# thekingofkings/embedding

Measured on AMD Instinct MI355X. Metric: SGNS training edges/sec, higher is better.
Workload: dtype f32

## Files before the change

embedding_amd/_native.py:

```python
import ctypes as C
import os

_HERE = os.path.dirname(os.path.abspath(__file__))
LIB_PATH = os.path.join(_HERE, "libdge.so")

DGE_OK, DGE_ERR_ARG, DGE_ERR_RANGE, DGE_ERR_TOPK, DGE_ERR_CAP, DGE_ERR_STATE, DGE_ERR_DEVICE, DGE_ERR_IO = range(8)


class DgeError(RuntimeError):
    def __init__(self, code, msg):
        super().__init__("libdge error %d: %s" % (code, msg))
        self.code = code


class TrainConfig(C.Structure):
    _fields_ = [
        ("dim", C.c_int32), ("window", C.c_int32), ("negative", C.c_int32), ("min_count", C.c_int32),
        ("epochs", C.c_int32), ("workers", C.c_int32), ("alpha", C.c_float), ("min_alpha", C.c_float),
        ("seed", C.c_uint64), ("table_size", C.c_int64), ("n_vertices", C.c_int32), ("update_policy", C.c_int32),
        ("use_hs", C.c_int32), ("reserved", C.c_int32),
    ]


class TrainStats(C.Structure):
# ... 242 lines not shown
    "dge_names_count": (_int, [_vp, _P(_i64)]),
    "dge_names_cstrs": (_int, [_vp, _P(_vp)]),
    "dge_names_free": (None, [_vp]),
    "dge_walks_from_seq_text": (_int, [_int, _vp, _i64, _vp, _int, _P(_vp), _P(SeqInfo)]),
    "dge_walks_from_seq_files": (_int, [_int, _vp, _i32, _vp, _int, _P(_vp), _P(SeqInfo)]),
    "dge_walks_to_seq_text": (_int, [_vp, _i64, _i64, _vp, _int, _vp, _i64, _P(_i64), _P(SeqOutInfo)]),
    "dge_walks_write_seq": (_int, [_vp, _i64, _i64, _vp, _int, C.c_char_p, _int, _P(SeqOutInfo)]),
    "dge_walks_to_host": (_int, [_vp, _vp, _i64]),
    "dge_walks_info": (_int, [_vp, _P(_i64), _P(_i32), _P(_vp)]),
    "dge_walks_add_position_prefix": (_int, [_vp, _i32]),
    "dge_walks_free": (None, [_vp]),
    "dge_count_tokens": (_int, [_vp, _i64, _i64, _i32, _vp]),
    "dge_model_create": (_int, [_int, _P(TrainConfig), _vp, _P(_vp)]),
    "dge_model_set_stream": (_int, [_vp, _vp]),
    "dge_model_train": (_int, [_vp, _vp, _i64, _i64, _i64, _i32, _i64, _dbl, _i64]),
    "dge_train_sgns": (_int, [_int, _vp, _i64, _i32, _P(TrainConfig), _P(_vp)]),
    "dge_train_sgns_device": (_int, [_vp, _P(TrainConfig), _P(_vp)]),
    "dge_model_walk_and_train": (_int, [_vp, _vp, _vp, _i64, _i64, _i64, _i64, _i32, _i64, _dbl, _i64]),
    "dge_model_vectors": (_int, [_vp, _P(_vp), _P(_vp), _P(_i64), _P(_i32)]),
    "dge_model_syn1neg": (_int, [_vp, _P(_vp)]),
    "dge_model_syn1": (_int, [_vp, _P(_vp), _P(_i64)]),
    "dge_model_huffman": (_int, [_vp, _P(_vp), _P(_vp), _P(_vp)]),
    "dge_model_counts": (_int, [_vp, _P(_vp)]),
    "dge_model_table": (_int, [_vp, _P(_vp), _P(_i64)]),
    "dge_model_stats": (_int, [_vp, _P(TrainStats)]),
    "dge_model_row_rates": (_int, [_vp, _P(C.c_double), _P(C.c_double), _P(C.c_double), _P(C.c_double)]),
    "dge_model_table_placement": (_int, [_vp, _i32, _vp, _vp, _vp]),
    "dge_model_table_runs": (_int, [_vp, _vp, _vp]),
    "dge_model_tune_placement": (_int, [_vp, _vp, _i64, _i64, _i32, _vp, _vp, _vp]),
    "dge_model_placement_search": (_int, [_vp, _vp, _vp, _vp, _vp]),
    "dge_model_reset_stats": (_int, [_vp]),
    "dge_model_schedule": (_int, [_vp, _P(_i32), _P(_i64), _P(_i32)]),
    "dge_model_kernel": (_int, [_vp, C.c_char_p, _i32]),
    "dge_model_lock_stats": (_int, [_vp, _P(_i64), _P(_i64), _P(_i64)]),
    "dge_model_score_pairs": (_int, [_vp, _vp, _vp, _i64, _vp]),
    "dge_model_eval_links": (_int, [_vp, _vp, _i64, _i64, _i32, C.c_uint64, _P(EvalResult)]),
    "dge_model_eval_sgns": (_int, [_vp, _vp, _i64, _i64, C.c_uint64, _P(EvalResult)]),
    "dge_write_vec": (_int, [_vp, _vp, C.c_char_p, _int]),
    "dge_model_free": (None, [_vp]),
    "dge_model_set_partition": (_int, [_vp, _i32, _i32, _i32]),
    "dge_model_partition_floats": (_int, [_vp, _i32, _P(_i64)]),
    "dge_model_export_partition": (_int, [_vp, _int, _i32, _i32, _vp]),
    "dge_model_import_partition": (_int, [_vp, _int, _i32, _i32, _vp]),
    "dge_model_export_partition_async": (_int, [_vp, _int, _i32, _i32, _vp, _vp]),
    "dge_model_import_partition_async": (_int, [_vp, _int, _i32, _i32, _vp, _vp]),
    "dge_model_stream": (_int, [_vp, _P(_vp)]),
    "dge_host_sync_count": (_int, [_P(_i64)]),
    "dge_model_sync_size": (_int, [_vp, _P(_i64)]),
    "dge_model_snapshot": (_int, [_vp]),
    "dge_model_export_delta": (_int, [_vp, _vp]),
    "dge_model_import_delta": (_int, [_vp, _vp, C.c_float]),
    "dge_comm_unique_id": (_int, [_vp]),
    "dge_comm_create": (_int, [_P(_vp), _vp, _int, _int, _int]),
    "dge_comm_free": (None, [_vp]),
    "dge_model_allreduce_deltas": (_int, [_vp, _vp]),
    "dge_model_ring_pass": (_int, [_vp, _vp, _i32]),
    "dge_model_gather_table": (_int, [_vp, _vp, _int]),
    "dge_set_tuning": (_int, [_i32, _i64]),
    "dge_get_tuning": (_int, [_i32, _vp]),
    "dge_ndcg_at_k": (_int, [_int, _vp, _i32, _vp, _i32, _i32, _i32, _P(_dbl), _P(_dbl)]),
    "dge_knn_cosine": (_int, [_int, _vp, _i32, _i32, _i32, _vp, _vp, _P(_dbl)]),
    "dge_vectors_from_vec_text": (_int, [_int, _vp, _i64, _int, _vp, _int, _P(_vp), _P(VecInfo)]),
    "dge_vectors_from_vec_files": (_int, [_int, _vp, _i32, _int, _vp, _int, _P(_vp), _P(VecInfo)]),
    "dge_vectors_from_host": (_int, [_int, _vp, _i64, _i32, _vp, _P(_vp)]),
    "dge_vectors_info": (_int, [_vp, _P(_i64), _P(_i32), _P(_vp), _P(_vp)]),
    "dge_vectors_to_host": (_int, [_vp, _vp, _vp, _i64]),
# ... 72 lines not shown
```

embedding_amd/csrc/sgns.hip:

```cpp
#include <hipcub/hipcub.hpp>
#include <math.h>
#include <stdlib.h>
#include <string.h>

#include <algorithm>
#include <limits>
#include <string>

#include "dge_algos.h"
#include "dge_internal.h"
#include "sgns_kernels.h"
#include "sgns_model.h"

std::atomic<int64_t> g_dge_tuning[DGE_TUNE_COUNT];
namespace { struct TuningInit { TuningInit() { for (auto& k : g_dge_tuning) k.store(-1); } } g_tuning_init; }
std::atomic<int64_t> g_dge_host_syncs{0};
extern "C" int dge_host_sync_count(int64_t* n) {
    if (!n) DGE_FAIL(DGE_ERR_ARG, "dge_host_sync_count: null output");
    *n = g_dge_host_syncs.load(std::memory_order_relaxed);
    return DGE_OK;
}
extern "C" int dge_set_tuning(int32_t knob, int64_t value) {
    if (knob < 0 || knob >= DGE_TUNE_COUNT) DGE_FAIL(DGE_ERR_ARG, "dge_set_tuning: unknown knob %d", knob);
    g_dge_tuning[knob] = value < 0 ? -1 : value;
// ... 584 lines not shown
    if (n_exceptions) *n_exceptions = m->n_exc;
    return DGE_OK;
}

extern "C" int dge_model_schedule(const dge_model* m, int32_t* update_policy, int64_t* workers, int32_t* hot_rows) {
    if (!m) DGE_FAIL(DGE_ERR_ARG, "dge_model_schedule: null model");
    if (!m->has_plan) DGE_FAIL(DGE_ERR_STATE, "dge_model_schedule: nothing has been trained yet");
    if (update_policy) *update_policy = m->last_plan.reported_policy();
    if (workers) *workers = m->last_plan.workers;
    if (hot_rows) *hot_rows = m->last_plan.hot_rows;
    return DGE_OK;
}

extern "C" int dge_model_lock_stats(const dge_model* mc, int64_t* pairs_put_back, int64_t* rounds_short, int64_t* rounds) {
    dge_model* m = const_cast<dge_model*>(mc);
    if (!m) DGE_FAIL(DGE_ERR_ARG, "dge_model_lock_stats: null model");
    DGE_HIP(hipSetDevice(m->device));
    DGE_HIP(hipStreamSynchronize(m->stream));
    unsigned long long c[3] = {0, 0, 0};
    DGE_HIP(hipMemcpy(c, m->d_counters + 4, sizeof(c), hipMemcpyDeviceToHost));
    if (pairs_put_back) *pairs_put_back = (int64_t)c[0];
    if (rounds_short) *rounds_short = (int64_t)c[1];
    if (rounds) *rounds = (int64_t)c[2];
    return DGE_OK;
}

extern "C" int dge_model_kernel(const dge_model* m, char* buf, int32_t cap) {
    if (!m || !buf || cap <= 0) DGE_FAIL(DGE_ERR_ARG, "dge_model_kernel: bad argument");
    if (!m->has_plan) DGE_FAIL(DGE_ERR_STATE, "dge_model_kernel: nothing has been trained yet");
    snprintf(buf, (size_t)cap, "%s", m->last_plan.kernel_name().c_str());
    return DGE_OK;
}

extern "C" int dge_model_reset_stats(dge_model* m) {
    if (!m) DGE_FAIL(DGE_ERR_ARG, "dge_model_reset_stats: null model");
    int rc = dge_drain_events(m);
    if (rc) return rc;
    DGE_HIP(hipMemsetAsync(m->d_counters, 0, 2 * sizeof(unsigned long long), m->stream));
    DGE_HIP(hipMemsetAsync(m->d_counters + 4, 0, 3 * sizeof(unsigned long long), m->stream));
    DGE_HIP(hipStreamSynchronize(m->stream));
    m->kernel_ms = 0; m->walk_ms = 0; m->launches = 0;
    return DGE_OK;
}

extern "C" int dge_model_set_partition(dge_model* m, int32_t n_parts, int32_t ctx_part, int32_t tgt_part) {
    if (!m) DGE_FAIL(DGE_ERR_ARG, "dge_model_set_partition: null model");
    if (n_parts <= 1) { m->part_n = 1; m->part_ctx = 0; m->part_tgt = 0; return DGE_OK; }
    if (ctx_part < 0 || ctx_part >= n_parts || tgt_part < 0 || tgt_part >= n_parts) DGE_FAIL(DGE_ERR_ARG, "dge_model_set_partition: partition out of range");
    if (m->V < n_parts) DGE_FAIL(DGE_ERR_ARG, "dge_model_set_partition: %d partitions for %lld vocabulary rows", n_parts, (long long)m->V);
    m->part_n = n_parts; m->part_ctx = ctx_part; m->part_tgt = tgt_part;
    return DGE_OK;
}
```

embedding_amd/csrc/sgns_kernels.h:

```cpp
#pragma once
#include <hip/hip_runtime.h>
#include <stdint.h>

#include "dge_algos.h"
#include "dge_internal.h"
#include "sgns_plan.h"

#define EXP_TABLE_SIZE 1000
#define MAX_EXP 6
#define NEG_BATCH 5

struct TrainParams {
    const int32_t* sen; const int64_t* len; const int64_t* wb;
    float* syn0; float* syn1neg;
    int32_t acc_rows, acc_drain;
    const uint4* ctab;
    const double* run_base; const uint32_t* run_row; const uint32_t* exc_slot; const int32_t* exc_row;
    int32_t n_runs, n_exc;
    double T_inv;
    const float* exp_table;
    int64_t n_rows; int32_t L, W, K, stride;
    int32_t D;
    int64_t V, T;
    uint64_t T_magic, W_magic;
// ... 1150 lines not shown
            l1.v[q].x += neu.v[q].x; l1.v[q].y += neu.v[q].y; l1.v[q].z += neu.v[q].z; l1.v[q].w += neu.v[q].w;
        }
        if (HOTMIX && (last < hot_rows || p.syn0_free)) {
            if (use_mb) lk_post<DCH>(s_mb, s_mb_flag, wk, n_posts, 2, lane == 0 ? last : -1, 1.0f, neu, lane);
            else rowA_atomic_axpy<DCH>(syn0, last, lane, 1.0f, neu);
        } else {
            rowA_store<DCH, 16, BIG>(l1, syn0, last, lane);
            row_commit_wait(STRICT ? row_probe_lines(syn0, last, lane, DCH * 2) : 0.f);
            if (lane == 14) row_unlock<STRICT>(locks0, last);
        }
        my_pairs++;
        if (PART) {
            pair_mask &= pair_mask - 1ull;
            c = first_bit_from(pair_mask, 0, c_hi + 1);
        } else {
            c++;
            if (c == i) c++;
        }
    }
    LK_CLOSE_CENTRE();
    if (pend_row >= 0 && !flushA_blocking<DCH, STRICT, BIG, HOTMIX>(syn1neg, locks1, pend_row, my_dh + (cur_buf ^ 1) * DCH * 64 + lane, lane, hot_rows, WD ? &s_deadline : nullptr)) LK_GIVE_UP();
#undef LK_TOK
#undef LK_POSITIVE
#undef LK_CLOSE_CENTRE
#undef LK_GIVE_UP
    if (lane == 0) {
        if (my_pairs) atomicAdd(&p.counters[0], my_pairs);
        if (my_words) atomicAdd(&p.counters[1], my_words);
        if (PART) { atomicAdd(&p.counters[4], (unsigned long long)n_aborted); atomicAdd(&p.counters[5], (unsigned long long)n_short); atomicAdd(&p.counters[6], (unsigned long long)n_rounds); }
        if (use_mb) __hip_atomic_fetch_add(&s_mb_done, 1, __ATOMIC_RELEASE, __HIP_MEMORY_SCOPE_WORKGROUP);
    }
}

#define HSW_NQ (DCH <= 2 ? 6 : 3)
template <int DCH>
__device__ __forceinline__ void hot_addA(float* s_hot, int* s_cnt, int slot, int drain, const TableView& t, int32_t row, int lane, const Row<DCH>& x) {
    float* a = s_hot + slot * (DCH * 64) + 4 * lane;
#pragma unroll
    for (int c = 0; c < DCH; c++) {
        atomicAdd(a + c * 64 + 0, x.v[c].x); atomicAdd(a + c * 64 + 1, x.v[c].y); atomicAdd(a + c * 64 + 2, x.v[c].z); atomicAdd(a + c * 64 + 3, x.v[c].w);
    }
    int n = 0;
    if (lane == 0) n = atomicAdd(&s_cnt[slot], 1) + 1;
    n = __shfl(n, 0, 16);
    if (n % drain == 0) {
        float* e = s_hot + slot * (DCH * 64) + lane;
        float* gp = t.base + (size_t)row * (t.row_bytes / 4) + lane;
#pragma unroll
        for (int c = 0; c < DCH; c++)
#pragma unroll
            for (int m = 0; m < 4; m++) {
                if ((uint32_t)(c * 64 + 16 * m + lane) >= t.valid) continue;
                const float v = atomicExch(e + c * 64 + 16 * m, 0.f);
                if (v != 0.f) atomicAdd(gp + c * 64 + 16 * m, v);
            }
    }
}
template <int DCH>
__device__ __forceinline__ void row_add(Row<DCH>& y, const Row<DCH>& x) {
#pragma unroll
    for (int c = 0; c < DCH; c++) { y.v[c].x += x.v[c].x; y.v[c].y += x.v[c].y; y.v[c].z += x.v[c].z; y.v[c].w += x.v[c].w; }
}
__device__ __forceinline__ int hsw_n_copies(const TrainParams& p, int32_t nd) {
    int r = 1;
#pragma unroll
    for (int k = 1; k < HS_REP; k++) r += nd >= p.hs_rep_thr[k] ? 1 : 0;
// ... 479 lines not shown
                else hipLaunchKernelGGL((k_sgns_train<DCH, 2, BIG, true, false>), g, b, pl.shmem, st, p);
            } else if (pl.part) hipLaunchKernelGGL((k_sgns_train<DCH, 2, BIG, false, true>), g, b, 0, st, p);
            else hipLaunchKernelGGL((k_sgns_train<DCH, 2, BIG, false, false>), g, b, 0, st, p);
            break;
        case TrainForm::HsCentre:
            if constexpr (DCH <= 4 && !BIG) {
                if (!pl.nlock) hipLaunchKernelGGL((k_sgns_train_hsw<DCH, false, 3>), g, b, pl.shmem, st, p);
                else if (pl.waves == 3) {
                    if (pl.head) hipLaunchKernelGGL((k_sgns_train_hsw<DCH, true, 3, true>), g, b, pl.shmem, st, p);
                    else hipLaunchKernelGGL((k_sgns_train_hsw<DCH, true, 3>), g, b, pl.shmem, st, p);
                } else if constexpr (DCH <= 2) {
                    if (pl.head) {
                        (void)hipFuncSetAttribute((const void*)k_sgns_train_hsw<DCH, true, 7, true>, hipFuncAttributeMaxDynamicSharedMemorySize, (int)pl.shmem);
                        hipLaunchKernelGGL((k_sgns_train_hsw<DCH, true, 7, true>), g, b, pl.shmem, st, p);
                    } else {
                        (void)hipFuncSetAttribute((const void*)k_sgns_train_hsw<DCH, true, 7>, hipFuncAttributeMaxDynamicSharedMemorySize, (int)pl.shmem);
                        hipLaunchKernelGGL((k_sgns_train_hsw<DCH, true, 7>), g, b, pl.shmem, st, p);
                    }
                }
            }
            break;
        case TrainForm::Locked:
            if (pl.hotmix) {
                if (pl.part) hipLaunchKernelGGL((k_sgns_train_locked<DCH, false, BIG, true, true>), g, b, 0, st, p);
                else hipLaunchKernelGGL((k_sgns_train_locked<DCH, false, BIG, true, false>), g, b, 0, st, p);
            } else if (pl.part) {
                if (pl.wdog) hipLaunchKernelGGL((k_sgns_train_locked<DCH, false, BIG, false, true, true>), g, b, 0, st, p);
                else hipLaunchKernelGGL((k_sgns_train_locked<DCH, false, BIG, false, true>), g, b, 0, st, p);
            } else if (pl.strict) {
                if (pl.wdog) hipLaunchKernelGGL((k_sgns_train_locked<DCH, true, BIG, false, false, true>), g, b, 0, st, p);
                else hipLaunchKernelGGL((k_sgns_train_locked<DCH, true, BIG, false, false>), g, b, 0, st, p);
            } else {
                if (pl.wdog) hipLaunchKernelGGL((k_sgns_train_locked<DCH, false, BIG, false, false, true>), g, b, 0, st, p);
                else hipLaunchKernelGGL((k_sgns_train_locked<DCH, false, BIG, false, false>), g, b, 0, st, p);
            }
            break;
        default: break;
    }
}
template <int DCH>
static inline void launch_train(const TrainParams& p, const TrainPlan& pl, hipStream_t st) {
    if (pl.big) launch_train_b<DCH, true>(p, pl, st);
    else launch_train_b<DCH, false>(p, pl, st);
}
```

embedding_amd/csrc/sgns_plan.h:

```cpp
#pragma once
#include <math.h>
#include <stdarg.h>
#include <stdint.h>
#include <stdio.h>

#include <algorithm>
#include <string>
#include <vector>

#include "../../include/dge.h"

#define HS_REP 16
#define HS_REP_NODES 64
#define HS_REP_ROWS ((HS_REP - 1) * HS_REP_NODES)
#ifndef DGE_LOCKED_WAVES
#define DGE_LOCKED_WAVES 3
#endif
#ifndef DGE_HOTMIX_WAVES
#define DGE_HOTMIX_WAVES 3
#endif
#ifndef DGE_HS_WAVES
#define DGE_HS_WAVES 3
#endif

// ... 73 lines not shown
    if (memo.n == n && memo.workers == W) return memo.rows;
    const double power = 0.75, twp = s.neg_norm, tw = (double)std::max<int64_t>(s.total_words, 1);
    double tail = 0.0; int64_t H = s.V;
    const double bound = 0.2 / (5.0 * (double)W * (double)std::max(n, 1));
    while (H > 0) {
        const double c = (double)counts[H - 1];
        const double q = pow(c, power) / twp, pp = c / tw;
        if (tail + q * q + pp * pp >= bound) break;
        tail += q * q + pp * pp; H--;
    }
    int64_t Hs = 0;
    while (Hs < s.V && (double)W * (double)n * (double)counts[Hs] / tw > 0.5) Hs++;
    memo.n = n; memo.workers = W; memo.rows = std::max(H, Hs);
    return memo.rows;
}

static inline double lock_failures(const ScheduleStats& s) { return (double)((int64_t)s.n_cus * 3 * 16) * 5.0 * s.neg_collision; }
static inline bool row_share_caps_workers(const ScheduleStats& s) { return (int64_t)(48.0 / std::max(s.row_share_max, 1e-12)) < 4096; }
static inline bool locks_work(const ScheduleStats& s) { return s.V >= 131072 && lock_failures(s) < 0.4; }
static inline bool tables_need_segments(const ScheduleStats& s) { return (uint64_t)s.V * (uint64_t)s.stride * 4ull >= 0xFFFFFFFFull; }
static inline bool big_tables(const ScheduleStats& s, const int64_t* knob) { return tables_need_segments(s) || knob[DGE_TUNE_FORCE_SEGMENTS] > 0; }

static inline bool syn1neg_locks_work(const ScheduleStats& s) { return !row_share_caps_workers(s) && locks_work(s); }
static inline int auto_policy(const ScheduleStats& s, bool hs) {
    if (hs) return 2;
    if (row_share_caps_workers(s)) return 2;
    if (locks_work(s)) return s.hot_rows_serial > 0 ? 7 : 5;
    if (s.V >= 131072 && s.hot_rows_auto <= s.V / 4) return 7;
    return 2;
}

static inline bool small_rows(const dge_train_config& cfg, const ScheduleStats& s, int policy, int part_n, int32_t L, bool big, const int64_t* knob) {
    return policy == 2 && cfg.use_hs == 0 && part_n <= 1 && cfg.dim > 16 && cfg.dim <= 32 && s.stride == 64 && L <= 64 && !big && knob[DGE_TUNE_SMALL_ROWS] != 0;
}

enum class TrainForm { Sorted, InOrder, RowRmw, Atomics, SmallRows, Locked, HsCentre };

struct TrainPlan {
    TrainForm form = TrainForm::InOrder;
    bool hs = false;
    bool part = false;
    bool strict = false;
    bool hotmix = false;
    bool wdog = false;
    bool nlock = false;
    bool head = false;
    int waves = 0;
    bool big = false;
    int64_t workers = 0;
    unsigned blocks = 0, threads = 0;
    size_t shmem = 0;
    int32_t hot_rows = 0, acc_rows = 0, acc_drain = 16, syn0_free = 0;
    int32_t hs_hot0 = 0x7fffffff, hs_n_hot = 0, hs_drain = 1, hs_cold = 0, hs_wave = 0, hs_rep0 = 0x7fffffff, hs_rep_n = 0;
    int32_t hs_rep_thr[HS_REP] = {0x7fffffff, 0x7fffffff, 0x7fffffff, 0x7fffffff, 0x7fffffff, 0x7fffffff, 0x7fffffff, 0x7fffffff,
                                  0x7fffffff, 0x7fffffff, 0x7fffffff, 0x7fffffff, 0x7fffffff, 0x7fffffff, 0x7fffffff, 0x7fffffff};
    uint64_t wd_ticks = 0;
    bool runs_off = false;
    bool walk_counter = false;
    char error[512] = "";

    int reported_policy() const {
        switch (form) {
            case TrainForm::Sorted: return 8;
            case TrainForm::InOrder: return 0;
            case TrainForm::RowRmw: return 1;
            case TrainForm::Locked: return hotmix ? 7 : (strict ? 6 : 5);
            case TrainForm::HsCentre: return nlock ? (head ? 7 : 5) : 2;
            default: return 2;
        }
    }
    std::string kernel_name() const {
        const std::string blk = part ? ", one block" : "";
        switch (form) {
            case TrainForm::Sorted:
                return part ? "k_sorted_phase (owner-computes, one block of the multi-GPU schedule: k_block_emit + 2 item sorts + 2 phases)"
                            : "k_sorted_phase (owner-computes: k_sorted_emit + 2 item sorts + 2 phases)";
            case TrainForm::HsCentre:
                if (!nlock) return "k_sgns_train_hsw<atomics, 3 waves> (hierarchical softmax, a wave per centre)";
                return std::string("k_sgns_train_hsw<negatives under commit locks") + (head ? ", head rows by atomics" : "") + (waves == 7 ? ", 7 waves>" : ", 3 waves>") +
                       " (hierarchical softmax, a wave per centre)";
            case TrainForm::Locked: return std::string("k_sgns_train_locked<") + (strict ? "strict" : "relaxed") + (hotmix ? ", head rows by atomics" : "") + blk + ">";
            case TrainForm::SmallRows: return "k_sgns_train_small<atomics, 32 lanes a worker>";
            default:
                return std::string("k_sgns_train<") + (form == TrainForm::Atomics ? "atomics" : (form == TrainForm::RowRmw ? "row rmw" : "in-order")) +
                       (hs ? ", hierarchical softmax pair by pair" : "") + blk + ">";
        }
    }
};

static inline int plan_fail(TrainPlan* out, int code, const char* fmt, ...) __attribute__((format(printf, 3, 4)));
static inline int plan_fail(TrainPlan* out, int code, const char* fmt, ...) {
// ... 151 lines not shown
            P.hs_cold = (int32_t)std::min<int64_t>(cold_knob >= 0 ? cold_knob : (int64_t)s.hs_cold_auto, P.hs_rep0);
        } else {
            const int64_t row_b = (int64_t)s.stride * 4 + 4;
            P.hs_n_hot = (int32_t)std::min<int64_t>(std::max<int64_t>(s.V - 1, 0), (hot_kb > 0 ? std::min<int64_t>(hot_kb, nw == 7 ? 100 : 30) * 1024 : (nw == 7 ? 15360 : 30720)) / row_b);
            P.hs_hot0 = (int32_t)(std::max<int64_t>(s.V - 1, 0) - P.hs_n_hot);
            P.hs_cold = (int32_t)std::min<int64_t>(cold_knob >= 0 ? cold_knob : (int64_t)s.hs_cold_auto, P.hs_hot0);
            P.shmem = (size_t)P.hs_n_hot * (size_t)row_b;
        }
    }
    if (P.form == TrainForm::Atomics && hs && workers > 1 && (knob[DGE_TUNE_HS_WAVE] > 0 || (knob[DGE_TUNE_HS_WAVE] < 0 && s.V >= 65536))) {
        P.hs_wave = 1;
        if (workers_auto) workers = std::max<int64_t>(std::min<int64_t>(workers / 16 * 12, (int64_t)s.n_cus * DGE_HS_WAVES * 12), 2);
        P.blocks = (unsigned)((workers + 11) / 12);
    }
    if (P.form == TrainForm::Locked && P.hotmix && workers > 1) {
        if (workers_auto) workers = std::max<int64_t>(workers / 16 * 12, 2);
        P.blocks = (unsigned)((workers + 11) / 12);
        if (part) P.acc_drain = knob[DGE_TUNE_ACC_DRAIN] > 0 ? (int32_t)std::min<int64_t>(knob[DGE_TUNE_ACC_DRAIN], 1 << 20)
                                                             : (int32_t)std::max<int64_t>(1, std::min<int64_t>(8, 2048 / std::max(P.blocks, 1u)));
    }
    P.workers = workers;
    P.big = big;
    const bool in_order = P.form == TrainForm::InOrder && !hs && !part;
    P.walk_counter = workers > 1 && n_rows >= 32 * workers && !in_order && !(knob[DGE_TUNE_STATIC_WALKS] > 0);
    P.runs_off = s.hot_rows_serial > 0 && workers > 1;
    {
        const double bytes = launch_pairs * 8.0 * (double)s.stride * (double)(cfg.negative + 2);
        double budget_s = 5.0 + 100.0 * bytes / 8e12;
        if (knob[DGE_TUNE_WATCHDOG_MS] > 0) budget_s = (double)knob[DGE_TUNE_WATCHDOG_MS] * 1e-3;
        const bool forced_locks = cfg.update_policy == 5 || cfg.update_policy == 6;
        P.wd_ticks = (!forced_locks || knob[DGE_TUNE_WATCHDOG_MS] == 0) ? 0ull : (uint64_t)(budget_s * 1e8);
    }
    P.wdog = P.form == TrainForm::Locked && !P.hotmix && P.wd_ticks != 0;
    if (small && P.form == TrainForm::Atomics && (workers > 1 || knob[DGE_TUNE_SMALL_ROWS] > 0)) {
        P.form = TrainForm::SmallRows;
        P.threads = 256u; P.blocks = (unsigned)((workers * 32 + 255) / 256);
    }
    return DGE_OK;
}
```

embedding_amd/engine.py:

```python
import ctypes as C
import os

import numpy as np

from ._native import DGE_COUNTS_PRESENT_ALL, DGE_COUNTS_PRESENT_NONZERO, DGE_ERR_CAP, DGE_FLOW_TEXT_MATRIX, DGE_FLOW_TEXT_OD, DGE_FLOW_TEXT_OD_LAYERED, DGE_SLOTS_AS_TRACTS, DGE_SLOTS_EVEN, CountsInfo, EvalResult, FlowSlices, FlowTextInfo, FlowsInfo, HourWindow, KmeansCfg, KmeansInfo, LocateInfo, MatrixReadInfo, MatrixReadOptions, OdInfo, RegionsInfo, RidgeInfo, SeqInfo, SeqOutInfo, SpatialInfo, SvmCfg, SvmInfo, TableReadInfo, TableReadOptions, TrainConfig, TrainStats, TreeCfg, TreeInfo, TripTextInfo, TripTextOptions, TripletInfo, TripletRule, VecInfo, check, lib
from .evaluate import _info_dict, _select_mask


def _ptr(a):
    return a.ctypes.data_as(C.c_void_p) if a is not None else None


_byref = C.byref


def _dev_ptr(t):
    if t is None:
        return None
    if isinstance(t, int):
        return C.c_void_p(t)
    return C.c_void_p(t.data_ptr())


class DeviceGraph:
# ... 1167 lines not shown
            n_rows = corpus.shape[0] - row0
        r = EvalResult()
        check(lib.dge_model_eval_sgns(self._h, corpus._h, int(row0), int(n_rows), int(seed), C.byref(r)))
        return self._eval_dict(r)

    def write_vec(self, path, names=None, header=False):
        arr = None
        if isinstance(names, Names):
            arr = names._cstrs()
        elif names is not None:
            arr = (C.c_char_p * len(names))(*[n.encode() if n is not None else None for n in names])
        check(lib.dge_write_vec(self._h, arr, str(path).encode(), int(bool(header))))

    def load_vectors(self, v):
        n = C.c_int64(0)
        check(lib.dge_model_load_vectors(self._h, v._h, C.byref(n)))
        return n.value

    def schedule(self):
        pol, w, hot = C.c_int32(0), C.c_int64(0), C.c_int32(0)
        check(lib.dge_model_schedule(self._h, C.byref(pol), C.byref(w), C.byref(hot)))
        return {"update_policy": pol.value, "workers": w.value, "hot_rows": hot.value}

    def lock_stats(self):
        a, b, c = C.c_int64(0), C.c_int64(0), C.c_int64(0)
        check(lib.dge_model_lock_stats(self._h, C.byref(a), C.byref(b), C.byref(c)))
        return {"pairs_put_back": a.value, "rounds_short": b.value, "rounds": c.value}

    def kernel(self):
        buf = C.create_string_buffer(256)
        check(lib.dge_model_kernel(self._h, buf, 256))
        return buf.value.decode()

    def set_partition(self, n_parts, ctx_part=0, tgt_part=0):
        check(lib.dge_model_set_partition(self._h, int(n_parts), int(ctx_part), int(tgt_part)))

    def partition_floats(self, n_parts):
        n = C.c_int64(0); check(lib.dge_model_partition_floats(self._h, int(n_parts), C.byref(n))); return n.value

    def export_partition(self, table, n_parts, part, d_buf):
        check(lib.dge_model_export_partition(self._h, int(table), int(n_parts), int(part), _dev_ptr(d_buf)))

    def import_partition(self, table, n_parts, part, d_buf):
        check(lib.dge_model_import_partition(self._h, int(table), int(n_parts), int(part), _dev_ptr(d_buf)))

    def export_partition_async(self, table, n_parts, part, d_buf, consumer_stream=0):
        check(lib.dge_model_export_partition_async(self._h, int(table), int(n_parts), int(part), _dev_ptr(d_buf), C.c_void_p(int(consumer_stream))))

    def import_partition_async(self, table, n_parts, part, d_buf, producer_stream=0):
        check(lib.dge_model_import_partition_async(self._h, int(table), int(n_parts), int(part), _dev_ptr(d_buf), C.c_void_p(int(producer_stream))))

    def stream(self):
        p = C.c_void_p(0); check(lib.dge_model_stream(self._h, C.byref(p))); return p.value or 0

    def sync_size(self):
        n = C.c_int64(0); check(lib.dge_model_sync_size(self._h, C.byref(n))); return n.value

    def snapshot(self):
        check(lib.dge_model_snapshot(self._h))

    def export_delta(self, d_buf):
        check(lib.dge_model_export_delta(self._h, _dev_ptr(d_buf)))

    def import_delta(self, d_buf, scale):
        check(lib.dge_model_import_delta(self._h, _dev_ptr(d_buf), float(scale)))

# ... 31 lines not shown
```

include/dge.h:

```cpp
#ifndef DGE_H
#define DGE_H
#include <stdint.h>

#ifdef __cplusplus
extern "C" {
#endif

#define DGE_VERSION 106

enum {
    DGE_OK = 0,
    DGE_ERR_ARG = 1,
    DGE_ERR_RANGE = 2,
    DGE_ERR_TOPK = 3,
    DGE_ERR_CAP = 4,
    DGE_ERR_STATE = 5,
    DGE_ERR_DEVICE = 6,
    DGE_ERR_IO = 7
};

typedef struct dge_graph dge_graph;
typedef struct dge_walks dge_walks;
typedef struct dge_model dge_model;

// ... 279 lines not shown
    int64_t words;
    double  kernel_ms;
    double  walk_kernel_ms;
    int64_t launches;
} dge_train_stats;

int  dge_count_tokens(const dge_walks* w, int64_t row0, int64_t n_rows, int32_t n_vertices, int64_t* d_counts);
int  dge_model_create(int device, const dge_train_config* cfg, const int64_t* d_counts, dge_model** out);
int  dge_model_set_stream(dge_model* m, void* hip_stream);
int  dge_model_train(dge_model* m, const dge_walks* w, int64_t row0, int64_t n_rows, int64_t walk_index_base,
                     int32_t epoch, int64_t words_before, double words_scale, int64_t total_walks_per_epoch);
int  dge_train_sgns(int device, const int32_t* walks , int64_t n_walks, int32_t max_len,
                    const dge_train_config* cfg, dge_model** out);
int  dge_train_sgns_device(const dge_walks* w, const dge_train_config* cfg, dge_model** out);
int  dge_model_walk_and_train(dge_model* m, const dge_graph* g, dge_walks* w, int64_t row0, int64_t n_rows,
                              int64_t walk_seed, int64_t walk_index_base, int32_t epoch, int64_t words_before,
                              double words_scale, int64_t total_walks_per_epoch);
int  dge_model_vectors(dge_model* m, const float** syn0, const int32_t** vocab_ids, int64_t* V, int32_t* dim);
int  dge_model_syn1neg(dge_model* m, const float** syn1neg);
int  dge_model_syn1(dge_model* m, const float** syn1, int64_t* rows);
int  dge_model_huffman(dge_model* m, const int64_t** offsets, const int32_t** points, const uint64_t** codes);
int  dge_model_counts(dge_model* m, const int64_t** counts);
int  dge_model_table(dge_model* m, const int32_t** table, int64_t* table_size);
int  dge_model_stats(const dge_model* m, dge_train_stats* out);
int  dge_model_row_rates(dge_model* m, double* read_gb_per_s, double* rewrite_gb_per_s, double* lock_exchanges_per_s, double* table_lookups_per_s);
int  dge_model_reset_stats(dge_model* m);
int  dge_model_table_placement(const dge_model* m, int32_t table, int32_t* candidates, double* best_gb_per_s, double* worst_gb_per_s);
int  dge_model_table_runs(const dge_model* m, int32_t* n_runs, int32_t* n_exceptions);
int  dge_model_tune_placement(dge_model* m, const dge_walks* w, int64_t row0, int64_t n_rows, int32_t candidates, double* ms_before, double* ms_after,
                              int32_t* arrays_moved);
int  dge_model_placement_search(const dge_model* m, int32_t* runs, double* ms_before, double* ms_after, int32_t* arrays_moved);
int  dge_model_schedule(const dge_model* m, int32_t* update_policy, int64_t* workers, int32_t* hot_rows);
int  dge_model_kernel(const dge_model* m, char* buf, int32_t cap);
int  dge_model_lock_stats(const dge_model* m, int64_t* pairs_put_back, int64_t* rounds_short, int64_t* rounds);
int  dge_host_sync_count(int64_t* n);
typedef struct dge_eval_result {
    int64_t pairs;
    int64_t negatives;
    int64_t skipped;
    double  auc;
    double  loss;
    double  kernel_ms;
} dge_eval_result;

int  dge_model_score_pairs(dge_model* m, const int32_t* d_ctx, const int32_t* d_tgt, int64_t n, float* d_score);

int  dge_model_eval_links(dge_model* m, const dge_walks* w, int64_t row0, int64_t n_rows,
                          int32_t regions_per_slice, uint64_t seed, dge_eval_result* out);

int  dge_model_eval_sgns(dge_model* m, const dge_walks* w, int64_t row0, int64_t n_rows,
                         uint64_t seed, dge_eval_result* out);

int  dge_write_vec(dge_model* m, const char* const* names, const char* path, int header);
void dge_model_free(dge_model* m);

int  dge_model_set_partition(dge_model* m, int32_t n_parts, int32_t ctx_part, int32_t tgt_part);
int  dge_model_partition_floats(const dge_model* m, int32_t n_parts, int64_t* n_floats);
int  dge_model_export_partition(dge_model* m, int table, int32_t n_parts, int32_t part, float* d_buf);
int  dge_model_import_partition(dge_model* m, int table, int32_t n_parts, int32_t part, const float* d_buf);
int  dge_model_export_partition_async(dge_model* m, int table, int32_t n_parts, int32_t part, float* d_buf, void* consumer_stream);
int  dge_model_import_partition_async(dge_model* m, int table, int32_t n_parts, int32_t part, const float* d_buf, void* producer_stream);
int  dge_model_stream(const dge_model* m, void** hip_stream);

int  dge_model_sync_size(const dge_model* m, int64_t* n_floats);
int  dge_model_snapshot(dge_model* m);
int  dge_model_export_delta(dge_model* m, float* d_buf);
// ... 293 lines not shown
```

Before: 992.2 million.

## Add LDS window kernel that accumulates per-walk syn0 deltas before flushing

Adds a locked SGNS kernel variant in which each block stages several walks in LDS slots and accumulates context-row (syn0) gradient deltas per walk position in shared memory. The summed deltas are flushed to global memory once, under row locks, after all centres of a walk finish, rather than doing a locked read-modify-write per pair. It also keeps a per-worker double-buffered syn1neg delta for the centre row. The planner selects it for non-strict locked runs at stride 128, or stride 64 under policy 5, when enough LDS slots fit. The cost is heavy LDS use with one block per CU, intra-block slot scheduling with spinning, and applying the syn0 updates later than before.

```diff
diff --git a/embedding_amd/_native.py b/embedding_amd/_native.py
--- a/embedding_amd/_native.py
+++ b/embedding_amd/_native.py
@@ -298,6 +298,7 @@
     "dge_model_reset_stats": (_int, [_vp]),
     "dge_model_schedule": (_int, [_vp, _P(_i32), _P(_i64), _P(_i32)]),
     "dge_model_kernel": (_int, [_vp, C.c_char_p, _i32]),
+    "dge_model_pair_loop": (_int, [_vp, _P(_i32), _P(_i32)]),
     "dge_model_lock_stats": (_int, [_vp, _P(_i64), _P(_i64), _P(_i64)]),
     "dge_model_score_pairs": (_int, [_vp, _vp, _vp, _i64, _vp]),
     "dge_model_eval_links": (_int, [_vp, _vp, _i64, _i64, _i32, C.c_uint64, _P(EvalResult)]),
diff --git a/embedding_amd/csrc/sgns.hip b/embedding_amd/csrc/sgns.hip
--- a/embedding_amd/csrc/sgns.hip
+++ b/embedding_amd/csrc/sgns.hip
@@ -640,6 +640,14 @@
     return DGE_OK;
 }
 
+extern "C" int dge_model_pair_loop(const dge_model* m, int32_t* loop, int32_t* slots) {
+    if (!m) DGE_FAIL(DGE_ERR_ARG, "dge_model_pair_loop: null model");
+    if (!m->has_plan) DGE_FAIL(DGE_ERR_STATE, "dge_model_pair_loop: nothing has been trained yet");
+    if (loop) *loop = m->last_plan.window ? 1 : 0;
+    if (slots) *slots = m->last_plan.window ? m->last_plan.win_slots : 0;
+    return DGE_OK;
+}
+
 extern "C" int dge_model_reset_stats(dge_model* m) {
     if (!m) DGE_FAIL(DGE_ERR_ARG, "dge_model_reset_stats: null model");
     int rc = dge_drain_events(m);
diff --git a/embedding_amd/csrc/sgns_kernels.h b/embedding_amd/csrc/sgns_kernels.h
--- a/embedding_amd/csrc/sgns_kernels.h
+++ b/embedding_amd/csrc/sgns_kernels.h
@@ -1206,6 +1206,391 @@
     }
 }
 
+
+#define WIN_WORKERS 48
+#define WIN_THREADS (WIN_WORKERS * 16)
+#define WIN_MAX_SLOTS 16
+#define WIN_CLOSED (1 << 24)
+#define WIN_FLUSH_LANES 13
+static_assert(WIN_WORKERS == DGE_WIN_WORKERS && WIN_MAX_SLOTS == DGE_WIN_MAX_SLOTS, "sgns_plan.h sizes the window's LDS");
+
+extern __shared__ __attribute__((aligned(16))) float s_win[];
+
+#define WIN_LD(x) __hip_atomic_load(&(x), __ATOMIC_RELAXED, __HIP_MEMORY_SCOPE_WORKGROUP)
+#define WIN_ST(x, v) __hip_atomic_store(&(x), (v), __ATOMIC_RELAXED, __HIP_MEMORY_SCOPE_WORKGROUP)
+
+__device__ __forceinline__ unsigned win_ballot16(bool b) { return (unsigned)(__ballot(b) >> (threadIdx.x & 48)) & 0xFFFFu; }
+
+template <int DCH>
+__device__ __forceinline__ void win_flush(const TableView& syn0, int* locks0, const float* sdelta, const int* stok, int len, int lane, int32_t filler_row) {
+    uint64_t pendm = len >= 2 ? (len >= 64 ? ~0ull : ((1ull << len) - 1ull)) : 0ull;
+    while (pendm) {
+        uint64_t m = pendm;
+        for (int j = 0; j < lane; j++) m &= m - 1ull;
+        const int pos = (lane < WIN_FLUSH_LANES && m) ? (int)__builtin_ctzll(m) : -1;
+        const int32_t row = pos >= 0 ? stok[pos] : -1;
+        const bool won = pos >= 0 ? row_trylock(locks0, row) : false;
+        const unsigned gotl = win_ballot16(won);
+        for (int base = 0; base < WIN_FLUSH_LANES; base += NEG_BATCH) {
+            const unsigned got = (gotl >> base) & ((1u << NEG_BATCH) - 1u);
+            if (!got) continue;
+            int32_t tg[NEG_BATCH];
+            int ps[NEG_BATCH];
+            Row<DCH> rr[NEG_BATCH];
+#pragma unroll
+            for (int q = 0; q < NEG_BATCH; q++) { tg[q] = __shfl(row, (base + q) & 15, 16); ps[q] = __shfl(pos, (base + q) & 15, 16); }
+#pragma unroll
+            for (int q = 0; q < NEG_BATCH; q++) rowA_load<DCH, 16, false>(rr[q], syn0, ((got >> q) & 1u) ? tg[q] : filler_row, lane);
+#pragma unroll
+            for (int q = 0; q < NEG_BATCH; q++)
+                if ((got >> q) & 1u) {
+                    const float* d = sdelta + ps[q] * (DCH * 64) + lane;
+#pragma unroll
+                    for (int k = 0; k < DCH; k++) {
+                        rr[q].v[k].x += d[k * 64]; rr[q].v[k].y += d[k * 64 + 16]; rr[q].v[k].z += d[k * 64 + 32]; rr[q].v[k].w += d[k * 64 + 48];
+                    }
+                    rowA_store<DCH, 16, false>(rr[q], syn0, tg[q], lane);
+                }
+        }
+        row_commit_wait(0.f);
+        if (won) row_unlock<false>(locks0, row);
+#pragma unroll
+        for (int j = 0; j < WIN_FLUSH_LANES; j++) {
+            const int pj = __shfl(pos, j, 16);
+            if ((gotl >> j) & 1u) pendm &= ~(1ull << pj);
+        }
+        if (pendm && !gotl) __builtin_amdgcn_s_sleep(2);
+    }
+}
+
+template <int DCH>
+__global__ void __launch_bounds__(WIN_THREADS, 1)
+k_sgns_train_window(TrainParams p, int n_slots) {
+    __shared__ float s_exp[EXP_TABLE_SIZE];
+    __shared__ double s_run_base[DGE_RUN_MAX];
+    __shared__ uint32_t s_run_row[DGE_RUN_MAX + 1];
+    __shared__ uint32_t s_exc_slot[DGE_RUN_EXC];
+    __shared__ int32_t s_exc_row[DGE_RUN_EXC];
+    __shared__ int s_next[WIN_MAX_SLOTS];
+    __shared__ int s_len[WIN_MAX_SLOTS];
+    __shared__ int s_done[WIN_MAX_SLOTS];
+    __shared__ int s_claim[WIN_MAX_SLOTS];
+    __shared__ int s_seq[WIN_MAX_SLOTS];
+    __shared__ float s_alpha[WIN_MAX_SLOTS];
+    __shared__ long long s_gbase[WIN_MAX_SLOTS];
+    __shared__ int s_seq_ctr, s_static_k, s_exhausted;
+    __shared__ unsigned s_plock[WIN_MAX_SLOTS * 2];
+
+    const bool use_runs = p.n_runs > 0;
+    if (use_runs) {
+        for (int i = threadIdx.x; i < DGE_RUN_MAX; i += blockDim.x) s_run_base[i] = p.run_base[i];
+        for (int i = threadIdx.x; i < DGE_RUN_MAX + 1; i += blockDim.x) s_run_row[i] = p.run_row[i];
+        for (int i = threadIdx.x; i < DGE_RUN_EXC; i += blockDim.x) { s_exc_slot[i] = p.exc_slot[i]; s_exc_row[i] = p.exc_row[i]; }
+    }
+    for (int i = threadIdx.x; i < EXP_TABLE_SIZE; i += blockDim.x) s_exp[i] = p.exp_table[i];
+    if (threadIdx.x < WIN_MAX_SLOTS) {
+        s_next[threadIdx.x] = WIN_CLOSED; s_len[threadIdx.x] = 0; s_done[threadIdx.x] = 0; s_seq[threadIdx.x] = 0;
+        s_claim[threadIdx.x] = (int)threadIdx.x < n_slots ? 0 : 1;
+    }
+    if (threadIdx.x < WIN_MAX_SLOTS * 2) s_plock[threadIdx.x] = 0u;
+    if (threadIdx.x == 0) { s_seq_ctr = 0; s_static_k = 0; s_exhausted = 0; }
+    __syncthreads();
+
+    const int lane = threadIdx.x & 15;
+    const int wk = threadIdx.x >> 4;
+    const int64_t worker = (int64_t)blockIdx.x * WIN_WORKERS + wk;
+    if (worker >= p.n_workers) return;
+
+    TableView syn0 = make_view(p.syn0, p.V, p.stride, p.big_seg_shift);
+    TableView syn1neg = make_view(p.syn1neg, p.V, p.stride, p.big_seg_shift);
+    syn0.valid = syn1neg.valid = (uint32_t)p.D;
+    int* const locks1 = p.locks;
+    int* const locks0 = p.locks + p.V + 1;
+
+    uint64_t mA = 1, cA = 0;
+    for (int j = 0; j <= lane; j++) { mA *= DGE_W2V_MULT; cA = cA * DGE_W2V_MULT + 11; }
+
+    const int L = p.L, W = p.W, K = p.K;
+    const int tok_pad = (L + 3) & ~3;
+    const int slot_floats = L * DCH * 64 + tok_pad;
+    float* const my_dh = s_win + (size_t)wk * 2 * DCH * 64;
+    float* const slots = s_win + (size_t)WIN_WORKERS * 2 * DCH * 64;
+    unsigned long long my_pairs = 0, my_words = 0;
+
+    int slot = 0, len = 0, i = 0, c = 1, c_hi = 0;
+    bool have = false;
+    int32_t word = 0;
+    float alpha = 0.f;
+    uint64_t s = 0;
+    Row<DCH> h;
+    bool h_dirty = false;
+    int32_t pend_row = -1;
+    int cur_buf = 0;
+    float* sdelta = slots;
+    const int* stok = (const int*)slots;
+
+#define WIN_POSITIVE()                                                                                                 \
+    do {                                                                                                               \
+        {      \
+            const float* sd_ = sdelta + c * (DCH * 64) + lane;                                                         \
+            _Pragma("unroll") for (int q_ = 0; q_ < DCH; q_++) {                                                       \
+                l1.v[q_].x += sd_[q_ * 64]; l1.v[q_].y += sd_[q_ * 64 + 16]; l1.v[q_].z += sd_[q_ * 64 + 32]; l1.v[q_].w += sd_[q_ * 64 + 48]; \
+            }                                                                                                          \
+        }                                                                                                              \
+        const float f_ = row_dot(l1, h);                                                                               \
+        const float g_ = sgns_g(f_, 1.0f, alpha, s_exp);                                                               \
+        row_axpy(neu, g_, h);                                                                                          \
+        row_axpy(h, g_, l1);                                                                                           \
+        float* d_ = my_dh + cur_buf * DCH * 64 + lane;                                                                 \
+        _Pragma("unroll") for (int q_ = 0; q_ < DCH; q_++) {                                                           \
+            d_[q_ * 64] = fmaf(g_, l1.v[q_].x, d_[q_ * 64]); d_[q_ * 64 + 16] = fmaf(g_, l1.v[q_].y, d_[q_ * 64 + 16]); \
+            d_[q_ * 64 + 32] = fmaf(g_, l1.v[q_].z, d_[q_ * 64 + 32]); d_[q_ * 64 + 48] = fmaf(g_, l1.v[q_].w, d_[q_ * 64 + 48]); \
+        }                                                                                                              \
+        h_dirty = true;                                                                                                \
+    } while (0)
+#define WIN_CLOSE_CENTRE()                                                                                             \
+    do {                                                                                                               \
+        if (h_dirty) {                                                                                                 \
+            h_dirty = false;                                                                                           \
+            if (pend_row >= 0) (void)flushA_blocking<DCH, false, false>(syn1neg, locks1, pend_row, my_dh + (cur_buf ^ 1) * DCH * 64 + lane, lane); \
+            pend_row = word; cur_buf ^= 1;                                                                             \
+        }                                                                                                              \
+    } while (0)
+
+    for (;;) {
+        bool new_centre = false;
+        if (c > c_hi) {
+            if (have) {
+                WIN_CLOSE_CENTRE();
+                have = false;
+                __builtin_amdgcn_fence(__ATOMIC_RELEASE, "workgroup");
+                int d = 0;
+                if (lane == 0) d = atomicAdd(&s_done[slot], 1) + 1;
+                d = __shfl(d, 0, 16);
+                if (d == len) {
+                    __builtin_amdgcn_fence(__ATOMIC_ACQUIRE, "workgroup");
+                    win_flush<DCH>(syn0, locks0, sdelta, stok, len, lane, p.filler_row);
+                    if (lane == 0) {
+                        WIN_ST(s_next[slot], WIN_CLOSED);
+                        __builtin_amdgcn_fence(__ATOMIC_RELEASE, "workgroup");
+                        WIN_ST(s_claim[slot], 0);
+                    }
+                }
+            }
+            int key = 0x7fffffff;
+            if (lane < n_slots) {
+                const int nx = WIN_LD(s_next[lane]), ln = WIN_LD(s_len[lane]);
+                if (nx < ln) key = (WIN_LD(s_seq[lane]) << 4) | lane;
+            }
+            key = min(key, __shfl_xor(key, 1, 16));
+            key = min(key, __shfl_xor(key, 2, 16));
+            key = min(key, __shfl_xor(key, 4, 16));
+            key = min(key, __shfl_xor(key, 8, 16));
+            if (key == 0x7fffffff) {
+                const bool mine = lane < n_slots;
+                const int cl = mine ? WIN_LD(s_claim[lane]) : 1;
+                const unsigned freem = win_ballot16(mine && cl == 0);
+                const unsigned loadm = win_ballot16(mine && cl != 0 && WIN_LD(s_next[lane]) >= WIN_CLOSED);
+                if (WIN_LD(s_exhausted)) {
+                    if (!loadm) break;
+                    __builtin_amdgcn_s_sleep(4);
+                    continue;
+                }
+                if (!freem) { __builtin_amdgcn_s_sleep(4); continue; }
+                const int f = __builtin_ctz(freem);
+                int ok = 0;
+                if (lane == 0) ok = atomicCAS(&s_claim[f], 0, 1) == 0 ? 1 : 0;
+                ok = __shfl(ok, 0, 16);
+                if (!ok) continue;
+                unsigned long long t = 0;
+                if (lane == 0) t = p.next_walk ? atomicAdd(p.next_walk, 1ull) : (unsigned long long)blockIdx.x + (unsigned long long)atomicAdd(&s_static_k, 1) * gridDim.x;
+                const int64_t w = (int64_t)shfl16_u64(t, 0);
+                int wl = 0;
+                if (w < p.n_rows) wl = min((int)p.len[w], L);
+                if (wl <= 0) {
+                    if (lane == 0) {
+                        if (w >= p.n_rows) WIN_ST(s_exhausted, 1);
+                        __builtin_amdgcn_fence(__ATOMIC_RELEASE, "workgroup");
+                        WIN_ST(s_claim[f], 0);
+                    }
+                    continue;
+                }
+                my_words += (unsigned long long)wl;
+                float* const sl_d = slots + (size_t)f * slot_floats;
+                int* const sl_t = (int*)(sl_d + L * DCH * 64);
+                const int32_t* sen = p.sen + w * L;
+                for (int j = lane; j < L; j += 16) sl_t[j] = j < wl ? sen[j] : -1;
+                for (int j = lane; j < wl * DCH * 16; j += 16) ((float4*)sl_d)[j] = make_float4(0.f, 0.f, 0.f, 0.f);
+                if (lane == 0) {
+                    const int64_t wbw = p.wb[w];
+                    const int64_t done = p.words_done_base + (p.words_scale == 1.0 ? wbw : (int64_t)((double)wbw * p.words_scale));
+                    float a = (float)((double)p.alpha0 * (1.0 - (double)done / (double)(p.all_words + 1)));
+                    if (a < p.min_alpha) a = p.min_alpha;
+                    s_alpha[f] = a;
+                    s_gbase[f] = (long long)((p.gidx_base + w) * (int64_t)L);
+                    s_len[f] = wl;
+                    s_done[f] = 0;
+                    s_seq[f] = atomicAdd(&s_seq_ctr, 1);
+                }
+                __builtin_amdgcn_fence(__ATOMIC_RELEASE, "workgroup");
+                if (lane == 0) WIN_ST(s_next[f], 0);
+                continue;
+            }
+            {
+                const int sl = key & 15;
+                int t = WIN_CLOSED;
+                if (lane == 0) t = atomicAdd(&s_next[sl], 1);
+                t = __shfl(t, 0, 16);
+                __builtin_amdgcn_fence(__ATOMIC_ACQUIRE, "workgroup");
+                const int ln = WIN_LD(s_len[sl]);
+                if (t >= ln) continue;
+                slot = sl; len = ln; i = t;
+            }
+            have = true;
+            sdelta = slots + (size_t)slot * slot_floats;
+            stok = (const int*)(sdelta + L * DCH * 64);
+            alpha = s_alpha[slot];
+            word = stok[i];
+            s = dge_mix64(p.seed + (uint64_t)((int64_t)s_gbase[slot] + i));
+            s = s * DGE_W2V_MULT + 11;
+            const int radius = W - (int)dge_fast_mod(s, (uint64_t)W, p.W_magic);
+            c = max(0, i - radius);
+            c_hi = min(len - 1, i + radius);
+            if (c_hi == i) c_hi--;
+            if (c == i) c++;
+            new_centre = true;
+            if (c > c_hi) continue;
+        }
+        const int32_t last = stok[c];
+
+        Row<DCH> l1, neu;
+        if (new_centre) {
+            if (pend_row == word) {
+                (void)flushA_blocking<DCH, false, false>(syn1neg, locks1, pend_row, my_dh + (cur_buf ^ 1) * DCH * 64 + lane, lane);
+                pend_row = -1;
+            }
+            rowA_load<DCH, 16, false>(h, syn1neg, word, lane);
+            float* d = my_dh + cur_buf * DCH * 64 + lane;
+#pragma unroll
+            for (int q = 0; q < DCH; q++) { d[q * 64] = 0.f; d[q * 64 + 16] = 0.f; d[q * 64 + 32] = 0.f; d[q * 64 + 48] = 0.f; }
+        }
+        rowA_load<DCH, 16, false>(l1, syn0, last, lane);
+        row_zero(neu);
+        bool have_l1 = false;
+        int kd = 0;
+        do {
+            const int kc = min(LK_CHUNK, K - kd);
+            int32_t t = -1;
+            {
+                const uint64_t sl = s * mA + cA;
+                if (lane < kc) {
+                    const uint64_t slt = dge_fast_mod(sl >> 16, (uint64_t)p.T, p.T_magic);
+                    t = use_runs ? neg_row_by_runs((uint32_t)slt, s_run_base, s_run_row, s_exc_slot, s_exc_row, p.n_exc, p.T_inv, p.V) : -2;
+                    if (t == -2) t = neg_table_row(p.ctab, slt);
+                    if (t == 0 && p.V > 1) t = (int32_t)(sl % (uint64_t)(p.V - 1)) + 1;
+                    if (t == word) t = -1;
+                }
+                if (kc > 0) s = shfl16_u64(sl, kc - 1);
+            }
+            if (lane == 13) t = pend_row;
+            unsigned pend13 = win_ballot16(lane < kc && t >= 0) & 0x1FFFu;
+            bool flush_pending = pend_row >= 0;
+            while (pend13 || !have_l1) {
+                const bool want = (lane < kc && ((pend13 >> lane) & 1u) && !(flush_pending && t == pend_row)) || (lane == 13 && flush_pending);
+                const bool won = want ? row_trylock(locks1, t) : false;
+                const unsigned gotl = win_ballot16(won);
+                const bool got_l1 = !have_l1;
+                const unsigned got13 = gotl & 0x1FFFu & pend13;
+                const bool gotf = flush_pending && ((gotl >> 13) & 1u);
+                Row<DCH> fr;
+                if (flush_pending) rowA_load<DCH, 16, false>(fr, syn1neg, gotf ? pend_row : p.filler_row, lane);
+                have_l1 = true;
+                bool do_pos = got_l1;
+                for (int base = 0; base < kc; base += NEG_BATCH) {
+                    const unsigned got = (got13 >> base) & ((1u << NEG_BATCH) - 1u);
+                    if (!got) continue;
+                    int32_t tg[NEG_BATCH];
+                    Row<DCH> rr[NEG_BATCH];
+#pragma unroll
+                    for (int q = 0; q < NEG_BATCH; q++) tg[q] = __shfl(t, (base + q) & 15, 16);
+#pragma unroll
+                    for (int q = 0; q < NEG_BATCH; q++) rowA_load<DCH, 16, false>(rr[q], syn1neg, ((got >> q) & 1u) ? tg[q] : p.filler_row, lane);
+                    if (do_pos) { do_pos = false; WIN_POSITIVE(); }
+#pragma unroll
+                    for (int q = 0; q < NEG_BATCH; q++)
+                        if ((got >> q) & 1u) {
+                            const float f = row_dot(l1, rr[q]);
+                            const float g = sgns_g(f, 0.0f, alpha, s_exp);
+                            row_axpy(neu, g, rr[q]);
+                            row_axpy(rr[q], g, l1);
+                            rowA_store<DCH, 16, false>(rr[q], syn1neg, tg[q], lane);
+                        }
+                }
+                if (do_pos) WIN_POSITIVE();
+                if (gotf) {
+                    const float* d = my_dh + (cur_buf ^ 1) * DCH * 64 + lane;
+#pragma unroll
+                    for (int q = 0; q < DCH; q++) {
+                        fr.v[q].x += d[q * 64]; fr.v[q].y += d[q * 64 + 16]; fr.v[q].z += d[q * 64 + 32]; fr.v[q].w += d[q * 64 + 48];
+                    }
+                    rowA_store<DCH, 16, false>(fr, syn1neg, pend_row, lane);
+                }
+                row_commit_wait(0.f);
+                if (won) row_unlock<false>(locks1, t);
+                pend13 &= ~got13;
+                if (gotf) { flush_pending = false; pend_row = -1; if (lane == 13) t = -1; }
+                if (pend13) __builtin_amdgcn_s_sleep(2);
+            }
+            kd += LK_CHUNK;
+        } while (kd < K);
+
+        {
+            float* sd = sdelta + c * (DCH * 64) + lane;
+            unsigned* const lw = &s_plock[slot * 2 + (c >> 5)];
+            const unsigned bit = 1u << (c & 31);
+            int got = 0;
+            if (lane == 0) got = (atomicOr(lw, bit) & bit) ? 0 : 1;
+            got = __shfl(got, 0, 16);
+            if (got) {
+                __builtin_amdgcn_fence(__ATOMIC_ACQUIRE, "workgroup");
+#pragma unroll
+                for (int q = 0; q < DCH; q++) {
+                    sd[q * 64] += neu.v[q].x; sd[q * 64 + 16] += neu.v[q].y; sd[q * 64 + 32] += neu.v[q].z; sd[q * 64 + 48] += neu.v[q].w;
+                }
+                __builtin_amdgcn_fence(__ATOMIC_RELEASE, "workgroup");
+                if (lane == 0) atomicAnd(lw, ~bit);
+            } else {
+                for (;;) {
+                    const bool won = lane == 0 ? row_trylock(locks0, last) : false;
+                    if (__shfl((int)won, 0, 16) != 0) {
+                        Row<DCH> cur;
+                        rowA_load<DCH, 16, false>(cur, syn0, last, lane);
+#pragma unroll
+                        for (int q = 0; q < DCH; q++) {
+                            cur.v[q].x += neu.v[q].x; cur.v[q].y += neu.v[q].y; cur.v[q].z += neu.v[q].z; cur.v[q].w += neu.v[q].w;
+                        }
+                        rowA_store<DCH, 16, false>(cur, syn0, last, lane);
+                        row_commit_wait(0.f);
+                        if (won) row_unlock<false>(locks0, last);
+                        break;
+                    }
+                    __builtin_amdgcn_s_sleep(2);
+                }
+            }
+        }
+        my_pairs++;
+        c++;
+        if (c == i) c++;
+    }
+    if (pend_row >= 0) (void)flushA_blocking<DCH, false, false>(syn1neg, locks1, pend_row, my_dh + (cur_buf ^ 1) * DCH * 64 + lane, lane);
+#undef WIN_POSITIVE
+#undef WIN_CLOSE_CENTRE
+    if (lane == 0) {
+        if (my_pairs) atomicAdd(&p.counters[0], my_pairs);
+        if (my_words) atomicAdd(&p.counters[1], my_words);
+    }
+}
+
 #define HSW_NQ (DCH <= 2 ? 6 : 3)
 template <int DCH>
 __device__ __forceinline__ void hot_addA(float* s_hot, int* s_cnt, int slot, int drain, const TableView& t, int32_t row, int lane, const Row<DCH>& x) {
@@ -1751,7 +2136,12 @@
                 else hipLaunchKernelGGL((k_sgns_train_locked<DCH, true, BIG, false, false>), g, b, 0, st, p);
             } else {
                 if (pl.wdog) hipLaunchKernelGGL((k_sgns_train_locked<DCH, false, BIG, false, false, true>), g, b, 0, st, p);
-                else hipLaunchKernelGGL((k_sgns_train_locked<DCH, false, BIG, false, false>), g, b, 0, st, p);
+                else if (pl.window) {
+                    if constexpr (DCH <= 2 && !BIG) {
+                        (void)hipFuncSetAttribute((const void*)k_sgns_train_window<DCH>, hipFuncAttributeMaxDynamicSharedMemorySize, (int)pl.win_shmem);
+                        hipLaunchKernelGGL((k_sgns_train_window<DCH>), dim3(pl.win_blocks), dim3(WIN_THREADS), pl.win_shmem, st, p, (int)pl.win_slots);
+                    }
+                } else hipLaunchKernelGGL((k_sgns_train_locked<DCH, false, BIG, false, false>), g, b, 0, st, p);
             }
             break;
         default: break;
diff --git a/embedding_amd/csrc/sgns_plan.h b/embedding_amd/csrc/sgns_plan.h
--- a/embedding_amd/csrc/sgns_plan.h
+++ b/embedding_amd/csrc/sgns_plan.h
@@ -129,6 +129,20 @@
 
 static inline bool small_rows(const dge_train_config& cfg, const ScheduleStats& s, int policy, int part_n, int32_t L, bool big, const int64_t* knob) {
     return policy == 2 && cfg.use_hs == 0 && part_n <= 1 && cfg.dim > 16 && cfg.dim <= 32 && s.stride == 64 && L <= 64 && !big && knob[DGE_TUNE_SMALL_ROWS] != 0;
+}
+
+#define DGE_LDS_BYTES 163840
+#define DGE_WIN_FIXED_BYTES 32768
+#define DGE_WIN_WORKERS 48
+#define DGE_WIN_MAX_SLOTS 16
+#define DGE_WIN_MIN_SLOTS 4
+static inline int64_t window_slot_bytes(int32_t stride, int32_t L) { return (int64_t)L * stride * 4 + (int64_t)((L + 3) & ~3) * 4; }
+static inline int window_slots(int32_t stride, int32_t L) {
+    const int64_t left = (int64_t)DGE_LDS_BYTES - DGE_WIN_FIXED_BYTES - (int64_t)DGE_WIN_WORKERS * 2 * stride * 4;
+    return (int)std::max<int64_t>(0, std::min<int64_t>(DGE_WIN_MAX_SLOTS, left / window_slot_bytes(stride, L)));
+}
+static inline size_t window_dyn_bytes(int32_t stride, int32_t L, int slots) {
+    return (size_t)((int64_t)DGE_WIN_WORKERS * 2 * stride * 4 + (int64_t)slots * window_slot_bytes(stride, L));
 }
 
 enum class TrainForm { Sorted, InOrder, RowRmw, Atomics, SmallRows, Locked, HsCentre };
@@ -154,6 +168,10 @@
     uint64_t wd_ticks = 0;
     bool runs_off = false;
     bool walk_counter = false;
+    bool window = false;
+    int32_t win_slots = 0;
+    unsigned win_blocks = 0;
+    size_t win_shmem = 0;
     char error[512] = "";
 
     int reported_policy() const {
@@ -371,6 +389,16 @@
         P.wd_ticks = (!forced_locks || knob[DGE_TUNE_WATCHDOG_MS] == 0) ? 0ull : (uint64_t)(budget_s * 1e8);
     }
     P.wdog = P.form == TrainForm::Locked && !P.hotmix && P.wd_ticks != 0;
+    const bool win_width = s.stride == 128 || (s.stride == 64 && cfg.update_policy == 5);
+    if (P.form == TrainForm::Locked && !P.strict && !P.hotmix && !part && !P.wdog && !big && win_width && workers > 1 && L >= 1 && L <= 64) {
+        const int slots = window_slots(s.stride, L);
+        if (slots >= DGE_WIN_MIN_SLOTS) {
+            P.window = true;
+            P.win_slots = slots;
+            P.win_blocks = (unsigned)std::min<int64_t>((workers + DGE_WIN_WORKERS - 1) / DGE_WIN_WORKERS, std::max(s.n_cus, 1));
+            P.win_shmem = window_dyn_bytes(s.stride, L, slots);
+        }
+    }
     if (small && P.form == TrainForm::Atomics && (workers > 1 || knob[DGE_TUNE_SMALL_ROWS] > 0)) {
         P.form = TrainForm::SmallRows;
         P.threads = 256u; P.blocks = (unsigned)((workers * 32 + 255) / 256);
diff --git a/embedding_amd/engine.py b/embedding_amd/engine.py
--- a/embedding_amd/engine.py
+++ b/embedding_amd/engine.py
@@ -1223,6 +1223,11 @@
         check(lib.dge_model_kernel(self._h, buf, 256))
         return buf.value.decode()
 
+    def pair_loop(self):
+        a, b = C.c_int32(0), C.c_int32(0)
+        check(lib.dge_model_pair_loop(self._h, C.byref(a), C.byref(b)))
+        return {"loop": a.value, "slots": b.value}
+
     def set_partition(self, n_parts, ctx_part=0, tgt_part=0):
         check(lib.dge_model_set_partition(self._h, int(n_parts), int(ctx_part), int(tgt_part)))
 
diff --git a/include/dge.h b/include/dge.h
--- a/include/dge.h
+++ b/include/dge.h
@@ -335,6 +335,7 @@
 int  dge_model_placement_search(const dge_model* m, int32_t* runs, double* ms_before, double* ms_after, int32_t* arrays_moved);
 int  dge_model_schedule(const dge_model* m, int32_t* update_policy, int64_t* workers, int32_t* hot_rows);
 int  dge_model_kernel(const dge_model* m, char* buf, int32_t cap);
+int  dge_model_pair_loop(const dge_model* m, int32_t* loop, int32_t* slots);
 int  dge_model_lock_stats(const dge_model* m, int64_t* pairs_put_back, int64_t* rounds_short, int64_t* rounds);
 int  dge_host_sync_count(int64_t* n);
 typedef struct dge_eval_result {
```

After: 1.056 billion (median of 6 runs). 1.06x the previous value.
